# Z2PackDev/TBmodels

Hardware: AMD Instinct MI355X
Metric: k-points/sec (H(k)+eig) at N_orb=64, N_R=4096 (higher is better)
Workload: dtype f64; 1 GPU; cfg2: dense N_orb=64 N_R=4096, 100000 random k-points per GPU, eigenval (H(k)+eig); kpoints_per_gpu=100000, collective=none, rccl_ranks=0, eigensolver=auto

## Files before the change

### tbmodels_amd/csrc/tbk_api.hip

```cpp

#include <algorithm>
#include <cmath>
#include <cstdarg>
#include <cstdlib>
#include <cstring>
#include <dlfcn.h>
#include <functional>
#include <new>
#include <vector>

#include "tbk_internal.h"

static thread_local char g_err[1024] = "";

void tbk_set_error(const char* fmt, ...) {
    va_list ap;
    va_start(ap, fmt);
    vsnprintf(g_err, sizeof(g_err), fmt, ap);
    va_end(ap);
}

extern "C" const char* tbk_last_error(void) { return g_err; }
#ifdef TBK_EXPERIMENTS
extern "C" const char* tbk_version(void) { return "tbk 0.1 (gfx950) +experiments"; }
// ... 283 lines not shown
            m->staged_bytes += nnz * (int64_t)(sizeof(int32_t) + 2 * sizeof(double));
            const int kt = tbk_csr_tile_kpoints(n_r);
            if (kt > 0) {
                std::vector<int64_t> sptr;
                std::vector<int32_t> srec_r;
                std::vector<double> srec_v;
                tbk_csr_schedule(m->ncol, kt, cptr, rec_r, rec_v, sptr, srec_r, srec_v);
                m->sched_steps = sptr.back();
                auto upload = [&](void** dst, const void* src, size_t bytes) -> int {
                    TBK_HIP(hipMalloc(dst, std::max<size_t>(bytes, 8)));
                    if (bytes) TBK_HIP(hipMemcpy(*dst, src, bytes, hipMemcpyHostToDevice));
                    m->staged_bytes += (int64_t)bytes;
                    return TBK_OK;
                };
                TBK_CHECK(upload((void**)&m->d_sptr, sptr.data(), sptr.size() * sizeof(int64_t)));
                TBK_CHECK(upload((void**)&m->d_srec_r, srec_r.data(), srec_r.size() * sizeof(int32_t)));
                TBK_CHECK(upload((void**)&m->d_srec_v, srec_v.data(), srec_v.size() * sizeof(double)));
                m->sched_kt = kt;
            }
        }
        return TBK_OK;
    }();
    if (rc != TBK_OK) {
        tbk_model_destroy(m);
        return rc;
    }
    *out = m;
    return TBK_OK;
}

extern "C" void tbk_model_destroy(tbk_model* m) {
    if (!m) return;
    (void)hipSetDevice(m->device);
    hipStream_t streams[] = {m->stream, m->stream_eig, m->stream_ql, m->stream_xl[0], m->stream_xl[1], m->stream_xl[2]};
    for (hipStream_t st : streams)
        if (st) (void)hipStreamSynchronize(st);
    for (hipEvent_t e : m->ev_xl)
        if (e) (void)hipEventDestroy(e);
    for (int b = 0; b < 2; ++b) {
        if (m->ev_hk[b]) (void)hipEventDestroy(m->ev_hk[b]);
        if (m->ev_tri[b]) (void)hipEventDestroy(m->ev_tri[b]);
        if (m->ev_ql[b]) (void)hipEventDestroy(m->ev_ql[b]);
        if (m->ev_out[b]) (void)hipEventDestroy(m->ev_out[b]);
        if (b == 0 && m->ev_sync) (void)hipEventDestroy(m->ev_sync);
    }
    for (auto& ev : m->events) {
        (void)hipEventDestroy(ev.start);
        (void)hipEventDestroy(ev.stop);
    }
    if (m->blas) (void)rocblas_destroy_handle(m->blas);
    if (m->h_stage) (void)hipHostFree(m->h_stage);
    for (hipStream_t st : streams)
        if (st) (void)hipStreamDestroy(st);
    void* ptrs[] = {m->d_R, m->d_colmap, m->d_B, m->d_cptr, m->d_rec_r, m->d_rec_v, m->d_powers, m->d_sptr, m->d_srec_r, m->d_srec_v};
    for (void* p : ptrs)
        if (p) (void)hipFree(p);
    DevBuf* bufs[] = {&m->ws_phase, &m->ws_H, &m->ws_E,   &m->ws_E2,
                      &m->ws_info,  &m->ws_k, &m->ws_pos, &m->ws_out, &m->ws_out2, &m->ws_flag, &m->ws_orb, &m->ws_part, &m->ws_kfold, &m->ws_kline, &m->ws_band, &m->ws_bandmat[0], &m->ws_bandmat[1], &m->ws_H2, &m->ws_split, &m->ws_xl, &m->ws_posraw};
    for (DevBuf* b : bufs) b->release();
    tbk_fold_release(m);
    delete m;
}

extern "C" int tbk_model_set_option(tbk_model* m, int option, int64_t value) {
    TBK_ARG(m != nullptr, "model is NULL");
    TBK_LOCK(m);
    switch (option) {
        case TBK_OPT_EIGENSOLVER:
            TBK_ARG(value >= TBK_EIG_AUTO && value <= TBK_EIG_ROCSOLVER, "unknown eigensolver");
            m->eigensolver = (int)value;
            return TBK_OK;
        case TBK_OPT_K_CHUNK:
            TBK_ARG(value >= 0, "k chunk must be >= 0");
            m->k_chunk = value;
            return TBK_OK;
        case TBK_OPT_TIMING:
            m->timing = value != 0;
            return TBK_OK;
        case TBK_OPT_FOLD:
            m->fold_enabled = value != 0;
            return TBK_OK;
        default:
            tbk_set_error("unknown option %d", option);
            return TBK_ERR_ARGUMENT;
    }
}

extern "C" int tbk_model_info(const tbk_model* m, int* device, int* dim, int* n_orb, int64_t* n_r,
                              int* is_sparse, int64_t* staged_bytes) {
    TBK_ARG(m != nullptr, "model is NULL");
    if (device) *device = m->device;
    if (dim) *dim = m->dim;
    if (n_orb) *n_orb = m->n_orb;
    if (n_r) *n_r = m->n_r;
    if (is_sparse) *is_sparse = m->sparse ? 1 : 0;
    if (staged_bytes) *staged_bytes = m->staged_bytes;
    return TBK_OK;
}

static int64_t choose_chunk(tbk_model* m, int64_t nk, bool with_eig) {
    if (nk <= TBK_BM) return TBK_BM;
    const int64_t n = m->n_orb;
    int64_t per_k = m->k2 * 8 + (with_eig ? n * n * 16 + (int64_t)tbk_eig_scratch_per_k(m) : 0);
    if (per_k < 64) per_k = 64;
    size_t free_b = 0, total_b = 0;
    if (hipMemGetInfo(&free_b, &total_b) != hipSuccess) free_b = size_t(8) << 30;
    free_b += m->ws_H.bytes + m->ws_H2.bytes + m->ws_phase.bytes + m->ws_band.bytes + m->ws_bandmat[0].bytes + m->ws_bandmat[1].bytes +
              m->ws_E.bytes + m->ws_xl.bytes;
    const bool mid = n > 64 && n <= 256;
    int64_t budget = std::min<int64_t>((int64_t)(free_b / 4), int64_t(mid ? 64 : n > 64 ? 24 : 6) << 30);
    int64_t chunk = budget / per_k / TBK_BM * TBK_BM;
    int64_t cap = mid ? 131072 : 32768;
    if (n < 64) cap *= std::min<int64_t>(32, (64 / n) * (64 / n));
    chunk = std::max<int64_t>(TBK_BM, std::min<int64_t>(chunk, cap));
    if (m->k_chunk > 0) chunk = round_up(m->k_chunk, TBK_BM);
    else if (chunk >= 4096) chunk = chunk / 4096 * 4096;
    return std::min(chunk, round_up(nk, TBK_BM));
}

static inline int64_t phase_ld(int64_t nk) { return round_up(nk, TBK_BM); }

static int fill_rows(tbk_model* m, const double* d_k, int64_t nk, int64_t nk_pad, double* d_A) {
    if (m->kdotp)
        return tbk_launch_monomials(m->stream, m->d_powers, m->dim, m->n_r, m->k2, d_k, nk, nk_pad, d_A);
    return tbk_launch_phase(m, d_k, nk, nk_pad, d_A);
}

static int build_h(tbk_model* m, const double* d_A, int64_t nk, int64_t nk_pad, int mode,
                   int convention, const double* d_k, const double* d_pos, double* d_H) {
    if (m->sparse)
        return tbk_launch_hk_csr(m, d_A, nk, nk_pad, mode, convention, d_k, d_pos, d_H);
    return tbk_launch_hk_dense(m, d_A, nk, nk_pad, mode, convention, d_k, d_pos, d_H);
}

extern "C" int tbk_hamilton_device(tbk_model* m, const double* d_k, int64_t nk, int convention,
                                   const double* d_pos, double* d_H) {
    TBK_ARG(m != nullptr, "model is NULL");
    TBK_LOCK(m);
    TBK_ARG(convention == 1 || convention == 2, "convention must be 1 or 2");
    TBK_ARG(nk >= 0, "nk < 0");
    if (nk == 0) return TBK_OK;
    TBK_ARG(d_k && d_H, "k / H is NULL");
    TBK_ARG(convention == 2 || d_pos != nullptr, "convention 1 needs pos");
    TBK_HIP(hipSetDevice(m->device));
    const int64_t chunk = choose_chunk(m, nk, false);
    const size_t nn2 = (size_t)m->n_orb * m->n_orb * 2;
    for (int64_t c0 = 0; c0 < nk; c0 += chunk) {
        const int64_t nkc = std::min(chunk, nk - c0);
        const int64_t nk_pad = phase_ld(nkc);
        TBK_CHECK(m->ws_phase.reserve((size_t)std::max<int64_t>(m->k2, 1) * nk_pad * sizeof(double)));
        double* d_A = m->ws_phase.as<double>();
        const double* kc = d_k + c0 * m->dim;
        const bool own_rows = tbk_hk_inline_phases(m, nkc);
        if (!own_rows) TBK_CHECK(fill_rows(m, kc, nkc, nk_pad, d_A));
        const double* d_orb = nullptr;
        const bool inline_orb = m->h_k_inline != nullptr && m->d_pos_inline != nullptr && nk == 1 && own_rows;
        if (convention == 1 && !inline_orb) {
            TBK_CHECK(m->ws_orb.reserve((size_t)nkc * m->n_orb * 2 * sizeof(double)));
            TBK_CHECK(tbk_launch_orbital_phases(m, kc, d_pos, nkc, m->ws_orb.as<double>()));
            d_orb = m->ws_orb.as<double>();
        }
// ... 853 lines not shown
```

### tbmodels_amd/csrc/tbk_hk_dense.hip

```cpp

#include <algorithm>
#include <cstdlib>
#include <type_traits>

#include "tbk_internal.h"

namespace {

typedef double d4 __attribute__((ext_vector_type(4)));
typedef double d2 __attribute__((ext_vector_type(2)));
typedef __attribute__((address_space(1))) const void* gptr_t;
typedef __attribute__((address_space(3))) void* lptr_t;

constexpr int LDA = TBK_BM + 16;
constexpr int LDB = 2 * TBK_BNP + 16;
constexpr int STAGE_DOUBLES = TBK_BK * (LDA + LDB);

static_assert(TBK_BM == 128 && TBK_BNP == 64 && TBK_BK == 16, "wave decomposition is written for 128x64x16");

struct HkArgs {
    const double* A;
    const double* Bt;
    const int32_t* colmap;
    const double* kpts;
    const int32_t* R;
    int64_t n_r;
    const double* pos;
    double* H;
    int64_t k2;
    int64_t nk;
    int64_t nk_pad;
    int ncol_pad;
    int n_orb;
    int dim;
    int mt_count;
    int nt_count;
    int xcd_rows;
    double* P;
    int splits;
    int unit_grid;
    int64_t p_rows;
    int64_t a_tile_stride;
    int64_t b_tile_stride;
    int rows_per_tile;
    int block_offset;
    int p_tiles;
    int sub_splits;
    double* P2;
    double k_val[TBK_MAX_DIM];
    int k_inline;
    const double* pos_raw;
};

__device__ __forceinline__ double hk_kcomp(const HkArgs& a, int64_t kq, int d) { return a.k_inline ? a.k_val[d] : a.kpts[kq * a.dim + d]; }

template <int MODE, int CONV>
__device__ __forceinline__ void store_element(const HkArgs& a, int64_t kq, int oi, int oj, double re, double im) {
    if (CONV == 1 && oi != oj) {
        d2 ei, ej;
        if (a.k_inline) {
            double di = 0.0, dj = 0.0;
            for (int d = 0; d < a.dim; ++d) {
                di = fma(a.k_val[d], a.pos_raw[oi * a.dim + d], di);
                dj = fma(a.k_val[d], a.pos_raw[oj * a.dim + d], dj);
            }
            double sn, cs;
            sincospi(2.0 * di, &sn, &cs);
            ei = (d2){cs, sn};
            sincospi(2.0 * dj, &sn, &cs);
            ej = (d2){cs, sn};
        } else {
            ei = *reinterpret_cast<const d2*>(a.pos + ((size_t)kq * a.n_orb + oi) * 2);
            ej = *reinterpret_cast<const d2*>(a.pos + ((size_t)kq * a.n_orb + oj) * 2);
        }
        const double cs = ei[0] * ej[0] + ei[1] * ej[1], sn = ei[0] * ej[1] - ei[1] * ej[0];
        const double t = re * cs - im * sn;
        im = re * sn + im * cs;
        re = t;
    }
    double* hk = a.H + (size_t)kq * a.n_orb * a.n_orb * 2;
    *reinterpret_cast<d2*>(hk + ((size_t)oi * a.n_orb + oj) * 2) = (d2){re, im};
    if (MODE == HK_FULL && oi != oj) *reinterpret_cast<d2*>(hk + ((size_t)oj * a.n_orb + oi) * 2) = (d2){re, -im};
}

__device__ __forceinline__ bool tile_of_block(const HkArgs& a, int b, int& mt, int& nt) {
    if (a.xcd_rows == 0) {
        nt = b % a.nt_count;
        mt = b / a.nt_count;
        return mt < a.mt_count;
    }
    const int x = b & 7;
    const int t = b >> 3;
    const int base = a.mt_count >> 3, extra = a.mt_count & 7;
    const int rows = base + (x < extra ? 1 : 0);
    if (t >= rows * a.nt_count) return false;
    const int start = x * base + (x < extra ? x : extra);
    const int full = rows / a.xcd_rows;
    const int per_group = a.xcd_rows * a.nt_count;
    int row;
    if (t < full * per_group) {
        const int g = t / per_group, r = t % per_group;
        row = g * a.xcd_rows + r % a.xcd_rows;
        nt = r / a.xcd_rows;
    } else {
        const int tt = t - full * per_group, rr = rows - full * a.xcd_rows;
        row = full * a.xcd_rows + tt % rr;
        nt = tt / rr;
    }
    mt = start + row;
    return true;
}

template <int MODE, int CONV, bool SPLIT>
__global__ void __launch_bounds__(256, 2) hk_dense_kernel(const HkArgs a) {
    extern __shared__ __attribute__((aligned(16))) double smem[];

    const int unit = (int)blockIdx.x + a.block_offset;
    const int split_y = SPLIT ? unit / a.unit_grid : 0;
    int mt_idx, nt_idx;
    if (!tile_of_block(a, SPLIT ? unit - split_y * a.unit_grid : unit, mt_idx, nt_idx)) return;

    const int tid = threadIdx.x;
    const int lane = tid & 63;
    const int wave = __builtin_amdgcn_readfirstlane(tid >> 6);
    const int wm = wave >> 1;
    const int wn = wave & 1;
    const int l15 = lane & 15;
    const int l4 = lane >> 4;

    const int64_t m0 = (int64_t)mt_idx * a.rows_per_tile;
    const int64_t n0 = (int64_t)nt_idx * TBK_BNP;

    d4 acc[4][2][2];
#pragma unroll
    for (int i = 0; i < 4; ++i)
// ... 481 lines not shown
int gemv_nkv(int64_t nk) {
    int nkv = 1;
    while (nkv < std::min<int64_t>(nk, 32)) nkv *= 2;
    return nkv;
}
int64_t gemv_strip_rows(const tbk_model* m, int64_t slices) {
    const int64_t n_pairs = m->k2 / 2;
    return (2 * ((n_pairs + slices - 1) / slices) + 15) / 16 * 16;
}

void gemv_plan(const tbk_model* m, int64_t nk, int* slices_out, size_t* lds_out) {
    const int nblk = m->ncol_pad / 64;
    const int64_t n_pairs = m->k2 / 2;
    const size_t per_split = (size_t)nk * m->ncol_pad * 2 * sizeof(double);
    const int64_t cap = std::max<int64_t>(1, (int64_t)((size_t(256) << 20) / per_split));
    const int64_t wave_slots = (int64_t)m->n_cu * 8;
    int64_t slices = wave_slots / nblk;
    size_t lds = 80 * 1024;
    const int64_t rows_one_round = slices > 0 ? (m->k2 + slices - 1) / slices : m->k2 + 1;
    if (slices < 1 || nblk * slices * 10 < wave_slots * 9 || rows_one_round > 384 || slices > cap) {
        slices = std::max<int64_t>(m->k2 / 256, std::min<int64_t>(((int64_t)m->n_cu * 32 + nblk - 1) / nblk, n_pairs / 8));
        slices = std::max<int64_t>(1, std::min(cap, slices));
        lds = 16 * 1024;
    }
    slices = std::max<int64_t>(1, std::min(slices, n_pairs / 8));
    if (nblk * slices * 2 <= wave_slots) lds = 16 * 1024;
    if (lds < 64 * 1024) {
        const size_t need = (size_t)4 * gemv_strip_rows(m, slices) * gemv_nkv(nk) * sizeof(double);
        if (need <= size_t(64) * 1024) lds = std::max(lds, need);
    }
    *slices_out = (int)slices;
    *lds_out = lds;
}

}

bool tbk_hk_inline_phases(const tbk_model* m, int64_t nk) {
    if (!tbk_hk_gemv_path(m, nk) || m->kdotp || m->d_R == nullptr) return false;
    int slices;
    size_t lds;
    gemv_plan(m, nk, &slices, &lds);
    return gemv_strip_rows(m, slices) * gemv_nkv(nk) <= (int64_t)(lds / 32);
}

bool tbk_hk_gemv_path(const tbk_model* m, int64_t nk) {
    if (nk < 1 || m->k2 <= 0 || m->sparse) return false;
    if (nk <= 32) return true;
    return nk <= 4096 && m->ncol_pad <= 256 && m->k2 < 16 * TBK_BK;
}

int tbk_launch_hk_dense(tbk_model* m, const double* d_A, int64_t nk, int64_t nk_pad, int mode,
                        int convention, const double* d_k, const double* d_pos, double* d_H) {
    if (nk == 0) return TBK_OK;
    HkArgs a;
    a.A = d_A;
    a.Bt = m->d_B;
    a.colmap = m->d_colmap;
    a.kpts = d_k;
    a.R = m->d_R;
    a.n_r = m->n_r;
    a.pos = d_pos;
    a.H = d_H;
    a.k2 = m->k2;
    a.nk = nk;
    a.nk_pad = nk_pad;
    a.ncol_pad = m->ncol_pad;
    a.n_orb = m->n_orb;
    a.dim = m->dim;
    a.mt_count = (int)((nk + TBK_BM - 1) / TBK_BM);
    a.nt_count = m->ncol_pad / TBK_BNP;
    int grid;
    if (a.mt_count >= 32) {
        a.xcd_rows = 4;
        if (const char* v = tbk_exp_env("TBK_HK_XCD_ROWS")) a.xcd_rows = std::max(1, atoi(v));
        const int max_rows = (a.mt_count + 7) / 8;
        grid = max_rows * a.nt_count * 8;
    } else {
        a.xcd_rows = 0;
        grid = a.mt_count * a.nt_count;
    }
    a.P = nullptr;
    a.splits = 1;
    a.p_rows = 0;
    a.a_tile_stride = TBK_BM;
    a.b_tile_stride = 0;
    a.rows_per_tile = TBK_BM;
    a.block_offset = 0;
    a.p_tiles = 0;
    a.sub_splits = 1;
    a.P2 = nullptr;
    a.unit_grid = 1;
    a.k_inline = 0;
    a.pos_raw = nullptr;
    for (int d = 0; d < TBK_MAX_DIM; ++d) a.k_val[d] = 0.0;
    if (tbk_hk_gemv_path(m, nk)) {
        int slices;
        size_t lds;
        gemv_plan(m, nk, &slices, &lds);
        const size_t per_split = (size_t)nk * a.ncol_pad * 2 * sizeof(double);
        if (m->h_k_inline != nullptr && nk == 1 && d_A == nullptr && tbk_hk_inline_phases(m, 1)) {
            a.k_inline = 1;
            for (int d = 0; d < m->dim; ++d) a.k_val[d] = m->h_k_inline[d];
            a.pos_raw = m->d_pos_inline;
        }
        TBK_ARG(d_A != nullptr || (tbk_hk_inline_phases(m, nk) && (d_k != nullptr || a.k_inline)), "phase rows missing");
        TBK_ARG(convention != 1 || mode == HK_TRI || d_pos != nullptr || (a.k_inline && a.pos_raw != nullptr), "convention 1 needs the orbital phases");
// ... 97 lines not shown
```

### tbmodels_amd/csrc/tbk_internal.h

```cpp
#pragma once

#include <hip/hip_runtime.h>
#include <rocblas/rocblas.h>

#include <atomic>
#include <cstdlib>
#include <cstdint>
#include <cstdio>
#include <functional>
#include <mutex>
#include <string>
#include <vector>

#include "tbk.h"

constexpr int TBK_BM = 128;
constexpr int TBK_BNP = 64;
constexpr int TBK_BK = 16;
constexpr int TBK_CT = 16;
constexpr int TBK_MAX_DIM = 8;

void tbk_set_error(const char* fmt, ...);

#define TBK_HIP(expr)                                                                             \
// ... 61 lines not shown
        return static_cast<T*>(ptr);
    }
};

struct EventPair {
    hipEvent_t start, stop;
    int stage;
};

struct tbk_fold_plan_t {
    bool built = false;
    int dim = 0;
    int64_t n_r = 0;
    int64_t n_rho = 0, n_rho_pad = 0, k2 = 0;
    int capacity = 0;
    std::vector<int32_t> h_R2;
    int32_t* d_R2 = nullptr;
    int64_t* d_lptr = nullptr;
    int32_t* d_lrec = nullptr;
    int32_t* d_rcomp = nullptr;
    double* d_B2 = nullptr;
    double* d_table = nullptr;
    int64_t table_entries = 0;
    tbk_fold_plan_t* sub = nullptr;
};

struct tbk_fold_saved_t {
    int dim;
    int64_t n_r, n_r_pad, k2;
    int32_t* d_R;
    double* d_B;
};

struct tbk_model {
    std::recursive_mutex mu;
    int device = 0;
    int64_t call_nk = 0;
    int n_cu = 256;
    int dim = 0;
    int n_orb = 0;
    int64_t n_r = 0;
    bool sparse = false;
    bool kdotp = false;

    int64_t n_r_pad = 0;
    int64_t k2 = 0;
    int ncol = 0;
    int ncol_pad = 0;
    int32_t* d_R = nullptr;
    int32_t* d_colmap = nullptr;
    int32_t* d_powers = nullptr;

    double* d_B = nullptr;

    int64_t nnz_rec = 0;
    int64_t* d_cptr = nullptr;
    int32_t* d_rec_r = nullptr;
    double* d_rec_v = nullptr;
    int sched_kt = 0;
    int64_t sched_steps = 0;
    int64_t* d_sptr = nullptr;
    int32_t* d_srec_r = nullptr;
    double* d_srec_v = nullptr;

    int64_t staged_bytes = 0;

    std::vector<int32_t> h_R;
    tbk_fold_plan_t fold[TBK_MAX_DIM];
    bool fold_enabled = true;
    int64_t counters[TBK_CNT_COUNT] = {0, 0, 0, 0};

    int eigensolver = TBK_EIG_AUTO;
    int64_t k_chunk = 0;
    bool timing = false;

    hipStream_t stream = nullptr;
    hipStream_t stream_eig = nullptr;
    hipStream_t stream_ql = nullptr;
    hipStream_t stream_xl[3] = {nullptr, nullptr, nullptr};
    hipEvent_t ev_xl[4] = {nullptr, nullptr, nullptr, nullptr};
    hipEvent_t ev_hk[2] = {nullptr, nullptr};
    hipEvent_t ev_tri[2] = {nullptr, nullptr};
    hipEvent_t ev_out[2] = {nullptr, nullptr};
    hipEvent_t ev_ql[2] = {nullptr, nullptr};
    hipEvent_t ev_sync = nullptr;
    rocblas_handle blas = nullptr;
    DevBuf ws_phase;
    DevBuf ws_H;
    DevBuf ws_H2;
    DevBuf ws_E;
    DevBuf ws_E2;
    DevBuf ws_info;
    DevBuf ws_k;
    DevBuf ws_pos;
    DevBuf ws_orb;
    DevBuf ws_out;
    DevBuf ws_out2;
    DevBuf ws_flag;
    void* h_stage = nullptr;
    size_t h_stage_bytes = 0;
    DevBuf ws_part;
    DevBuf ws_kfold;
    DevBuf ws_kline;
    DevBuf ws_band;
    DevBuf ws_bandmat[2];
    const double* h_k_inline = nullptr;
    const double* d_pos_inline = nullptr;
    std::vector<double> pos_cache;
    DevBuf ws_posraw;
    DevBuf ws_split;
    DevBuf ws_xl;
    std::function<int(int64_t c0, int64_t nkc, hipEvent_t done)> chunk_done;
    size_t hk_lds_floor = 0;
    std::vector<EventPair> events;
    double t_ms[TBK_T_COUNT] = {0, 0, 0, 0};
    int64_t t_n[TBK_T_COUNT] = {0, 0, 0, 0};
};

struct tbk_kdotp {
    tbk_model* core = nullptr;
};

void tbk_range_push(const char* name);
void tbk_range_pop();

struct StageTimer {
    tbk_model* m;
    EventPair ev;
    bool on;
    hipStream_t stream;
    StageTimer(tbk_model* m_, int stage, hipStream_t s = nullptr);
    ~StageTimer();
};

enum HkMode { HK_TRI = 0, HK_FULL = 1 };

int tbk_launch_phase(tbk_model* m, const double* d_k, int64_t nk, int64_t nk_pad, double* d_A);
int tbk_launch_orbital_phases(tbk_model* m, const double* d_k, const double* d_pos, int64_t nk, double* d_orb);
int tbk_launch_monomials(hipStream_t s, const int32_t* d_powers, int dim, int64_t n_p,
                         int64_t n_p_pad, const double* d_k, int64_t nk, int64_t nk_pad,
                         double* d_A);

int tbk_stage_dense(tbk_model* m, const double* d_hop_raw);
int tbk_stage_kdotp(tbk_model* m, const double* d_coeff_raw);

int tbk_launch_hk_dense(tbk_model* m, const double* d_A, int64_t nk, int64_t nk_pad, int mode,
                        int convention, const double* d_k, const double* d_pos, double* d_H);

int tbk_launch_hk_dense_lines(tbk_model* m, const double* d_A, int64_t n_lines, int line_len, int64_t b_stride, double* d_H);

int tbk_launch_hk_csr(tbk_model* m, const double* d_A, int64_t nk, int64_t nk_pad, int mode,
                      int convention, const double* d_k, const double* d_pos, double* d_H);

int tbk_csr_tile_kpoints(int64_t n_r);
void tbk_csr_schedule(int ncol, int kt, const std::vector<int64_t>& cptr, const std::vector<int32_t>& rec_r, const std::vector<double>& rec_v,
                      std::vector<int64_t>& sptr, std::vector<int32_t>& srec_r, std::vector<double>& srec_v);

int tbk_eig_batched(tbk_model* m, double* d_H, int64_t nk, double* d_E);

bool tbk_eig_stream_supported(int n);
int tbk_launch_tridiag_stream(tbk_model* m, hipStream_t s, double* d_H, int64_t nk, double* d_de, int method = 0);
bool tbk_hk_inline_phases(const tbk_model* m, int64_t nk);
bool tbk_hk_gemv_path(const tbk_model* m, int64_t nk);
int tbk_launch_bisect(tbk_model* m, hipStream_t s, const double* d_de, int64_t nk, double* d_E);
size_t tbk_eig_scratch_per_k(const tbk_model* m);
int tbk_band_xl_reserve(tbk_model* m, int64_t max_nk);

bool tbk_eig_band_supported(int n);
bool tbk_eig_band_preferred(int n);
size_t tbk_band_scratch_per_matrix(int n);
size_t tbk_band_bytes_per_matrix(int n);
size_t tbk_band_xl_buffer_per_matrix(int n);
bool tbk_eig_two_stage(const tbk_model* m);
int tbk_launch_band_reduce(tbk_model* m, hipStream_t s, double* d_H, int64_t nk, void* d_vw, void* d_band,
                           double* d_de_fused = nullptr);
bool tbk_band_fused(int n);
bool tbk_band_split(const tbk_model* m, int64_t nk);
bool tbk_band_xl_grouped(int n, int64_t nk);
int tbk_launch_band_chase(tbk_model* m, hipStream_t s, const void* d_band, int64_t nk, double* d_de);

bool tbk_eig_small_supported(int n);
int tbk_launch_tridiag(tbk_model* m, hipStream_t s, double* d_H, int64_t nk, double* d_de);
bool tbk_eig_reg128_supported(int n);
int tbk_launch_tridiag_reg128(hipStream_t s, double* d_H, int n, int64_t nk, double* d_D, double* d_E, int64_t h_stride, int ldd, int off);
int tbk_launch_tridiag_tail64(hipStream_t s, double* d_H, int64_t nk, double* d_D, double* d_E, int n_full, int64_t call_nk);
int tbk_launch_ql(tbk_model* m, hipStream_t s, const double* d_de, int64_t nk, double* d_E, bool beside_ql = false);

int tbk_fold_choose(tbk_model* m, const double* h_k, int64_t nk, std::vector<int64_t>& run_starts);
int tbk_fold_group_size();
int tbk_fold_group(tbk_model* m, tbk_fold_plan_t& plan, const double* h_kf, int n_g, int slot0);
int tbk_fold_lines(tbk_model* m, tbk_fold_plan_t& plan, const double* d_kf, int64_t stride, int n_lines, int slot0 = 0);
int tbk_fold_enter(tbk_model* m, tbk_fold_plan_t& plan, int slot, tbk_fold_saved_t& saved);
void tbk_fold_leave(tbk_model* m, const tbk_fold_saved_t& saved);
int tbk_fold_drop_component(tbk_model* m, const double* d_k, int dim, int f, int64_t nk, double* d_k2);
int tbk_fold_subplan(tbk_model* m, tbk_fold_plan_t& parent, int f2, int capacity, tbk_fold_plan_t** out);
void tbk_fold_release(tbk_model* m);
int64_t tbk_fold_min_run();

int tbk_run_mfma_f64_peak(double* tflops);
```

### tbmodels_amd/csrc/tbk_phase.hip

```cpp

#include "tbk_internal.h"

namespace {

__global__ void __launch_bounds__(256)
phase_rows_kernel(const double* __restrict__ k, const int32_t* __restrict__ R, int dim, int64_t nk,
                  int64_t nk_pad, int64_t n_r, double* __restrict__ A) {
    const int64_t kidx = (int64_t)blockIdx.x * blockDim.x + threadIdx.x;
    const int64_t r = blockIdx.y;
    if (kidx >= nk_pad) return;
    double c = 0.0, s = 0.0;
    if (kidx < nk && r < n_r) {
        double dot = 0.0;
        for (int d = 0; d < dim; ++d)
            dot = fma(k[kidx * dim + d], (double)R[r * dim + d], dot);
        sincospi(2.0 * dot, &s, &c);
    }
    A[(2 * r) * nk_pad + kidx] = c;
    A[(2 * r + 1) * nk_pad + kidx] = s;
}

__global__ void __launch_bounds__(256)
monomial_rows_kernel(const double* __restrict__ k, const int32_t* __restrict__ powers, int dim,
                     int64_t nk, int64_t nk_pad, int64_t n_p, double* __restrict__ A) {
    const int64_t kidx = (int64_t)blockIdx.x * blockDim.x + threadIdx.x;
    const int64_t p = blockIdx.y;
    if (kidx >= nk_pad) return;
    double v = 0.0;
    if (kidx < nk && p < n_p) {
        v = 1.0;
        for (int d = 0; d < dim; ++d) {
            const double x = k[kidx * dim + d];
            const int e = powers[p * dim + d];
            double acc = 1.0;
            for (int t = 0; t < e; ++t) acc *= x;
            v *= acc;
        }
    }
    A[p * nk_pad + kidx] = v;
}

__global__ void __launch_bounds__(256)
orbital_phase_kernel(const double* __restrict__ k, const double* __restrict__ pos, int dim, int64_t nk,
                     int n_orb, double* __restrict__ orb) {
    const int64_t idx = (int64_t)blockIdx.x * blockDim.x + threadIdx.x;
    if (idx >= nk * n_orb) return;
    const int64_t kq = idx / n_orb;
    const int p = (int)(idx % n_orb);
    double dot = 0.0;
    for (int d = 0; d < dim; ++d) dot = fma(k[kq * dim + d], pos[p * dim + d], dot);
    double s, c;
    sincospi(2.0 * dot, &s, &c);
    orb[2 * idx] = c;
    orb[2 * idx + 1] = s;
}

}

int tbk_launch_orbital_phases(tbk_model* m, const double* d_k, const double* d_pos, int64_t nk, double* d_orb) {
    if (nk == 0) return TBK_OK;
    const int64_t total = nk * m->n_orb;
    hipLaunchKernelGGL(orbital_phase_kernel, dim3((unsigned)((total + 255) / 256)), dim3(256), 0, m->stream, d_k,
                       d_pos, m->dim, nk, m->n_orb, d_orb);
    TBK_HIP(hipGetLastError());
    return TBK_OK;
}

int tbk_launch_phase(tbk_model* m, const double* d_k, int64_t nk, int64_t nk_pad, double* d_A) {
    if (m->n_r_pad == 0 || nk_pad == 0) return TBK_OK;
    StageTimer t(m, TBK_T_PHASE);
    dim3 grid((unsigned)((nk_pad + 255) / 256), (unsigned)m->n_r_pad);
    hipLaunchKernelGGL(phase_rows_kernel, grid, dim3(256), 0, m->stream, d_k, m->d_R, m->dim, nk,
                       nk_pad, m->n_r, d_A);
    TBK_HIP(hipGetLastError());
    return TBK_OK;
}

int tbk_launch_monomials(hipStream_t s, const int32_t* d_powers, int dim, int64_t n_p,
                         int64_t n_p_pad, const double* d_k, int64_t nk, int64_t nk_pad,
                         double* d_A) {
    if (n_p_pad == 0 || nk_pad == 0) return TBK_OK;
    dim3 grid((unsigned)((nk_pad + 255) / 256), (unsigned)n_p_pad);
    hipLaunchKernelGGL(monomial_rows_kernel, grid, dim3(256), 0, s, d_k, d_powers, dim, nk, nk_pad,
                       n_p, d_A);
    TBK_HIP(hipGetLastError());
    return TBK_OK;
}
```

### tbmodels_amd/csrc/tbk_stage.hip

```cpp

#include "tbk_internal.h"

namespace {

__global__ void __launch_bounds__(256)
stage_dense_kernel(const double* __restrict__ hop, const int32_t* __restrict__ colmap, int n_orb,
                   int64_t n_r, int ncol_pad, double* __restrict__ Bt) {
    const int e = blockIdx.x * blockDim.x + threadIdx.x;
    const int64_t r = blockIdx.y;
    if (e >= ncol_pad || r >= n_r) return;
    const int32_t ij = colmap[e];
    if (ij < 0) return;
    const int i = ij >> 16, j = ij & 0xffff;
    const double* blk = hop + (size_t)r * n_orb * n_orb * 2;
    const double hr = blk[((size_t)i * n_orb + j) * 2], hi = blk[((size_t)i * n_orb + j) * 2 + 1];
    const double gr = blk[((size_t)j * n_orb + i) * 2], gi = blk[((size_t)j * n_orb + i) * 2 + 1];
    const size_t tiles = ncol_pad / TBK_CT;
    const size_t base0 = (((size_t)(2 * r) * tiles + e / TBK_CT) * 2) * TBK_CT + e % TBK_CT;
    const size_t base1 = (((size_t)(2 * r + 1) * tiles + e / TBK_CT) * 2) * TBK_CT + e % TBK_CT;
    Bt[base0] = hr + gr;
    Bt[base0 + TBK_CT] = hi - gi;
    Bt[base1] = -(hi + gi);
    Bt[base1 + TBK_CT] = hr - gr;
}

__global__ void __launch_bounds__(256)
stage_kdotp_kernel(const double* __restrict__ coeff, const int32_t* __restrict__ colmap, int n_orb,
                   int64_t n_p, int ncol_pad, double* __restrict__ Bt) {
    const int e = blockIdx.x * blockDim.x + threadIdx.x;
    const int64_t p = blockIdx.y;
    if (e >= ncol_pad || p >= n_p) return;
    const int32_t ij = colmap[e];
    if (ij < 0) return;
    const int i = ij >> 16, j = ij & 0xffff;
    const double* blk = coeff + (size_t)p * n_orb * n_orb * 2;
    const size_t tiles = ncol_pad / TBK_CT;
    const size_t base = (((size_t)p * tiles + e / TBK_CT) * 2) * TBK_CT + e % TBK_CT;
    Bt[base] = blk[((size_t)i * n_orb + j) * 2];
    Bt[base + TBK_CT] = blk[((size_t)i * n_orb + j) * 2 + 1];
}

}

int tbk_stage_dense(tbk_model* m, const double* d_hop_raw) {
    const size_t bytes = (size_t)m->k2 * m->ncol_pad * 2 * sizeof(double);
    if (bytes == 0) return TBK_OK;
    TBK_HIP(hipMalloc((void**)&m->d_B, bytes));
    m->staged_bytes += (int64_t)bytes;
    TBK_HIP(hipMemsetAsync(m->d_B, 0, bytes, m->stream));
    if (m->n_r > 0) {
        TBK_ARG(m->n_r <= 65535, "more than 65535 lattice vectors");
        dim3 grid((m->ncol_pad + 255) / 256, (unsigned)m->n_r);
        hipLaunchKernelGGL(stage_dense_kernel, grid, dim3(256), 0, m->stream, d_hop_raw, m->d_colmap,
                           m->n_orb, m->n_r, m->ncol_pad, m->d_B);
        TBK_HIP(hipGetLastError());
    }
    return TBK_OK;
}

int tbk_stage_kdotp(tbk_model* m, const double* d_coeff_raw) {
    const size_t bytes = (size_t)m->k2 * m->ncol_pad * 2 * sizeof(double);
    if (bytes == 0) return TBK_OK;
    TBK_HIP(hipMalloc((void**)&m->d_B, bytes));
    m->staged_bytes += (int64_t)bytes;
    TBK_HIP(hipMemsetAsync(m->d_B, 0, bytes, m->stream));
    if (m->n_r > 0) {
        TBK_ARG(m->n_r <= 65535, "more than 65535 Taylor coefficients");
        dim3 grid((m->ncol_pad + 255) / 256, (unsigned)m->n_r);
        hipLaunchKernelGGL(stage_kdotp_kernel, grid, dim3(256), 0, m->stream, d_coeff_raw,
                           m->d_colmap, m->n_orb, m->n_r, m->ncol_pad, m->d_B);
        TBK_HIP(hipGetLastError());
    }
    return TBK_OK;
}
```

Baseline: 961,000 k-points/s.

## Emulate the FP64 H(k) GEMM with int8 MFMA over sixteen CRT moduli

```diff
diff --git a/tbmodels_amd/csrc/tbk_api.hip b/tbmodels_amd/csrc/tbk_api.hip
--- a/tbmodels_amd/csrc/tbk_api.hip
+++ b/tbmodels_amd/csrc/tbk_api.hip
@@ -359,11 +359,11 @@
     if (m->h_stage) (void)hipHostFree(m->h_stage);
     for (hipStream_t st : streams)
         if (st) (void)hipStreamDestroy(st);
-    void* ptrs[] = {m->d_R, m->d_colmap, m->d_B, m->d_cptr, m->d_rec_r, m->d_rec_v, m->d_powers, m->d_sptr, m->d_srec_r, m->d_srec_v};
+    void* ptrs[] = {m->d_R, m->d_colmap, m->d_B, m->d_Bres, m->d_bexp, m->d_cptr, m->d_rec_r, m->d_rec_v, m->d_powers, m->d_sptr, m->d_srec_r, m->d_srec_v};
     for (void* p : ptrs)
         if (p) (void)hipFree(p);
     DevBuf* bufs[] = {&m->ws_phase, &m->ws_H, &m->ws_E,   &m->ws_E2,
-                      &m->ws_info,  &m->ws_k, &m->ws_pos, &m->ws_out, &m->ws_out2, &m->ws_flag, &m->ws_orb, &m->ws_part, &m->ws_kfold, &m->ws_kline, &m->ws_band, &m->ws_bandmat[0], &m->ws_bandmat[1], &m->ws_H2, &m->ws_split, &m->ws_xl, &m->ws_posraw};
+                      &m->ws_info,  &m->ws_k, &m->ws_pos, &m->ws_out, &m->ws_out2, &m->ws_flag, &m->ws_orb, &m->ws_part, &m->ws_kfold, &m->ws_kline, &m->ws_band, &m->ws_bandmat[0], &m->ws_bandmat[1], &m->ws_H2, &m->ws_split, &m->ws_xl, &m->ws_posraw, &m->ws_ares, &m->ws_planes};
     for (DevBuf* b : bufs) b->release();
     tbk_fold_release(m);
     delete m;
@@ -413,7 +413,7 @@
     size_t free_b = 0, total_b = 0;
     if (hipMemGetInfo(&free_b, &total_b) != hipSuccess) free_b = size_t(8) << 30;
     free_b += m->ws_H.bytes + m->ws_H2.bytes + m->ws_phase.bytes + m->ws_band.bytes + m->ws_bandmat[0].bytes + m->ws_bandmat[1].bytes +
-              m->ws_E.bytes + m->ws_xl.bytes;
+              m->ws_E.bytes + m->ws_xl.bytes + m->ws_ares.bytes + m->ws_planes.bytes;
     const bool mid = n > 64 && n <= 256;
     int64_t budget = std::min<int64_t>((int64_t)(free_b / 4), int64_t(mid ? 64 : n > 64 ? 24 : 6) << 30);
     int64_t chunk = budget / per_k / TBK_BM * TBK_BM;
diff --git a/tbmodels_amd/csrc/tbk_hk_dense.hip b/tbmodels_amd/csrc/tbk_hk_dense.hip
--- a/tbmodels_amd/csrc/tbk_hk_dense.hip
+++ b/tbmodels_amd/csrc/tbk_hk_dense.hip
@@ -56,8 +56,8 @@
 
 template <int MODE, int CONV>
 __device__ __forceinline__ void store_element(const HkArgs& a, int64_t kq, int oi, int oj, double re, double im) {
+    d2 ei = (d2){1.0, 0.0}, ej = (d2){1.0, 0.0};
     if (CONV == 1 && oi != oj) {
-        d2 ei, ej;
         if (a.k_inline) {
             double di = 0.0, dj = 0.0;
             for (int d = 0; d < a.dim; ++d) {
@@ -73,14 +73,8 @@
             ei = *reinterpret_cast<const d2*>(a.pos + ((size_t)kq * a.n_orb + oi) * 2);
             ej = *reinterpret_cast<const d2*>(a.pos + ((size_t)kq * a.n_orb + oj) * 2);
         }
-        const double cs = ei[0] * ej[0] + ei[1] * ej[1], sn = ei[0] * ej[1] - ei[1] * ej[0];
-        const double t = re * cs - im * sn;
-        im = re * sn + im * cs;
-        re = t;
-    }
-    double* hk = a.H + (size_t)kq * a.n_orb * a.n_orb * 2;
-    *reinterpret_cast<d2*>(hk + ((size_t)oi * a.n_orb + oj) * 2) = (d2){re, im};
-    if (MODE == HK_FULL && oi != oj) *reinterpret_cast<d2*>(hk + ((size_t)oj * a.n_orb + oi) * 2) = (d2){re, -im};
+    }
+    tbk_store_h_element<MODE, CONV>(a.H, a.n_orb, kq, oi, oj, re, im, ei[0], ei[1], ej[0], ej[1]);
 }
 
 __device__ __forceinline__ bool tile_of_block(const HkArgs& a, int b, int& mt, int& nt) {
@@ -668,6 +662,7 @@
 int tbk_launch_hk_dense(tbk_model* m, const double* d_A, int64_t nk, int64_t nk_pad, int mode,
                         int convention, const double* d_k, const double* d_pos, double* d_H) {
     if (nk == 0) return TBK_OK;
+    if (tbk_hk_i8_route(m, nk)) return tbk_launch_hk_i8(m, d_k, nk, mode, convention, d_pos, d_H);
     HkArgs a;
     a.A = d_A;
     a.Bt = m->d_B;
diff --git a/tbmodels_amd/csrc/tbk_hk_i8.hip b/tbmodels_amd/csrc/tbk_hk_i8.hip
--- /dev/null
+++ b/tbmodels_amd/csrc/tbk_hk_i8.hip
@@ -0,0 +1,369 @@
+
+#include <cmath>
+#include <cstdlib>
+
+#include "tbk_internal.h"
+
+namespace {
+
+__constant__ int c_mod[TBK_I8_NMOD] = {256, 255, 253, 251, 247, 241, 239, 233, 229, 227, 223, 217, 211, 199, 197, 193};
+constexpr int H_MOD[TBK_I8_NMOD] = {256, 255, 253, 251, 247, 241, 239, 233, 229, 227, 223, 217, 211, 199, 197, 193};
+constexpr int ALPHA = 52;
+
+typedef int v4i __attribute__((ext_vector_type(4)));
+typedef int v16i __attribute__((ext_vector_type(16)));
+typedef double d2 __attribute__((ext_vector_type(2)));
+
+constexpr int I8_BN = 128;
+constexpr int I8_LDR = 80;
+constexpr int I8_STAGE = (TBK_I8_BM + I8_BN) * I8_LDR;
+static_assert(TBK_I8_BM == 256 && TBK_I8_BK == 64, "wave decomposition is written for 256 x 128 x 64");
+
+constexpr int modinv(int a, int p) {
+    a %= p;
+    for (int x = 1; x < p; ++x)
+        if ((a * x) % p == 1) return x;
+    return 0;
+}
+
+template <int P>
+__device__ __forceinline__ int sym(int r) {
+    return 2 * r >= P ? r - P : r;
+}
+
+__device__ __forceinline__ int sym_mod_f64(double x, int p) {
+    const double q = floor(x * (1.0 / (double)p));
+    int r = (int)fma(-q, (double)p, x);
+    if (r < 0) r += p;
+    if (r >= p) r -= p;
+    return 2 * r >= p ? r - p : r;
+}
+
+__global__ void __launch_bounds__(256)
+i8_stage_kernel(const double* __restrict__ Bt, int nc, int64_t k2, int64_t kpad, int beta, int8_t* __restrict__ Bres,
+                int32_t* __restrict__ bexp, int* __restrict__ nonfinite) {
+    __shared__ double s_max[256];
+    const int c = blockIdx.x;
+    double mx = 0.0;
+    bool bad = false;
+    for (int64_t kk = threadIdx.x; kk < k2; kk += 256) {
+        const double v = Bt[kk * nc + c];
+        mx = fmax(mx, fabs(v));
+        bad |= !isfinite(v);
+    }
+    if (bad) atomicAdd(nonfinite, 1);
+    s_max[threadIdx.x] = mx;
+    __syncthreads();
+    for (int w = 128; w > 0; w >>= 1) {
+        if (threadIdx.x < w) s_max[threadIdx.x] = fmax(s_max[threadIdx.x], s_max[threadIdx.x + w]);
+        __syncthreads();
+    }
+    mx = s_max[0];
+    int ex = 0;
+    if (mx > 0.0) (void)frexp(mx, &ex);
+    const int bc = mx > 0.0 ? beta - ex : 0;
+    if (threadIdx.x == 0) bexp[c] = bc;
+    for (int64_t kk = threadIdx.x; kk < kpad; kk += 256) {
+        const double v = kk < k2 && mx > 0.0 ? rint(ldexp(Bt[kk * nc + c], bc)) : 0.0;
+        const int64_t iv = isfinite(v) ? (int64_t)v : 0;
+#pragma unroll
+        for (int i = 0; i < TBK_I8_NMOD; ++i) {
+            const int p = c_mod[i];
+            int r = (int)(iv % p);
+            if (r < 0) r += p;
+            Bres[((int64_t)i * nc + c) * kpad + kk] = (int8_t)(2 * r >= p ? r - p : r);
+        }
+    }
+}
+
+__global__ void __launch_bounds__(256)
+i8_rows_kernel(const double* __restrict__ k, const int32_t* __restrict__ R, int dim, int64_t nk, int64_t n_r, int64_t mpad,
+               int64_t kpad, int8_t* __restrict__ Ares, int* __restrict__ row_bad) {
+    const int64_t r = (int64_t)blockIdx.x * blockDim.x + threadIdx.x;
+    const int64_t m = blockIdx.y;
+    if (2 * r >= kpad) return;
+    double c = 0.0, s = 0.0;
+    if (m < nk && r < n_r) {
+        double dot = 0.0;
+        for (int d = 0; d < dim; ++d) dot = fma(k[m * dim + d], (double)R[r * dim + d], dot);
+        sincospi(2.0 * dot, &s, &c);
+        if (!isfinite(c) || !isfinite(s)) {
+            row_bad[m] = 1;
+            c = s = 0.0;
+        }
+    }
+    const double ca = rint(ldexp(c, ALPHA)), sa = rint(ldexp(s, ALPHA));
+#pragma unroll
+    for (int i = 0; i < TBK_I8_NMOD; ++i) {
+        const int p = c_mod[i];
+        const uint32_t lo = (uint32_t)(uint8_t)(int8_t)sym_mod_f64(ca, p), hi = (uint32_t)(uint8_t)(int8_t)sym_mod_f64(sa, p);
+        *reinterpret_cast<uint16_t*>(Ares + ((int64_t)i * mpad + m) * kpad + 2 * r) = (uint16_t)(lo | (hi << 8));
+    }
+}
+
+template <int I>
+__device__ __forceinline__ int mod_pick(int x, int z) {
+    if constexpr (I == TBK_I8_NMOD) {
+        return 0;
+    } else {
+        if (z == I) {
+            int r = x % H_MOD[I];
+            return r < 0 ? r + H_MOD[I] : r;
+        }
+        return mod_pick<I + 1>(x, z);
+    }
+}
+
+__global__ void __launch_bounds__(256, 2)
+hk_i8_gemm_kernel(const int8_t* __restrict__ Ares, const int8_t* __restrict__ Bres, uint8_t* __restrict__ planes, int64_t mpad,
+                  int nc, int64_t kpad, int nt_count) {
+    extern __shared__ __attribute__((aligned(16))) char smem_i8[];
+    const int z = blockIdx.z;
+    const int mt = blockIdx.x / nt_count, nt = blockIdx.x - mt * nt_count;
+    const int tid = threadIdx.x, lane = tid & 63;
+    const int wave = __builtin_amdgcn_readfirstlane(tid >> 6);
+    const int wm = wave >> 1, wn = wave & 1;
+    const int l31 = lane & 31, l5 = lane >> 5;
+
+    const int8_t* gA = Ares + ((int64_t)z * mpad + (int64_t)mt * TBK_I8_BM) * kpad;
+    const int8_t* gB = Bres + ((int64_t)z * nc + (int64_t)nt * I8_BN) * kpad;
+    const int prow = tid >> 2, ppart = (tid & 3) * 16;
+    v4i ra[4], rb[2];
+    auto fetch = [&](int64_t kb) {
+#pragma unroll
+        for (int s = 0; s < 4; ++s) ra[s] = *reinterpret_cast<const v4i*>(gA + (int64_t)(prow + 64 * s) * kpad + kb + ppart);
+#pragma unroll
+        for (int s = 0; s < 2; ++s) rb[s] = *reinterpret_cast<const v4i*>(gB + (int64_t)(prow + 64 * s) * kpad + kb + ppart);
+    };
+    auto put = [&](int buf) {
+        char* sA = smem_i8 + buf * I8_STAGE;
+        char* sB = sA + TBK_I8_BM * I8_LDR;
+#pragma unroll
+        for (int s = 0; s < 4; ++s) *reinterpret_cast<v4i*>(sA + (prow + 64 * s) * I8_LDR + ppart) = ra[s];
+#pragma unroll
+        for (int s = 0; s < 2; ++s) *reinterpret_cast<v4i*>(sB + (prow + 64 * s) * I8_LDR + ppart) = rb[s];
+    };
+
+    v16i acc[4][2];
+#pragma unroll
+    for (int i = 0; i < 4; ++i)
+#pragma unroll
+        for (int j = 0; j < 2; ++j)
+#pragma unroll
+            for (int r = 0; r < 16; ++r) acc[i][j][r] = 0;
+
+    const int n_stage = (int)(kpad / TBK_I8_BK);
+    fetch(0);
+    put(0);
+    __syncthreads();
+    for (int st = 0; st < n_stage; ++st) {
+        const int buf = st & 1;
+        if (st + 1 < n_stage) fetch((int64_t)(st + 1) * TBK_I8_BK);
+        const char* sA = smem_i8 + buf * I8_STAGE + (wm * 128 + l31) * I8_LDR + l5 * 16;
+        const char* sB = smem_i8 + buf * I8_STAGE + TBK_I8_BM * I8_LDR + (wn * 64 + l31) * I8_LDR + l5 * 16;
+#pragma unroll
+        for (int ks = 0; ks < 2; ++ks) {
+            v4i fa[4], fb[2];
+#pragma unroll
+            for (int i = 0; i < 4; ++i) fa[i] = *reinterpret_cast<const v4i*>(sA + i * 32 * I8_LDR + ks * 32);
+#pragma unroll
+            for (int j = 0; j < 2; ++j) fb[j] = *reinterpret_cast<const v4i*>(sB + j * 32 * I8_LDR + ks * 32);
+#pragma unroll
+            for (int i = 0; i < 4; ++i)
+#pragma unroll
+                for (int j = 0; j < 2; ++j) acc[i][j] = __builtin_amdgcn_mfma_i32_32x32x32_i8(fa[i], fb[j], acc[i][j], 0, 0, 0);
+        }
+        if (st + 1 < n_stage) put(buf ^ 1);
+        __syncthreads();
+    }
+
+    uint8_t* out = planes + ((int64_t)z * mpad + (int64_t)mt * TBK_I8_BM + wm * 128) * nc + (int64_t)nt * I8_BN + wn * 64;
+#pragma unroll
+    for (int i = 0; i < 4; ++i)
+#pragma unroll
+        for (int j = 0; j < 2; ++j)
+#pragma unroll
+            for (int r = 0; r < 16; ++r)
+                out[(int64_t)(i * 32 + (r & 3) + 8 * (r >> 2) + 4 * l5) * nc + j * 32 + l31] = (uint8_t)mod_pick<0>(acc[i][j][r], z);
+}
+
+template <int I, int J>
+__device__ __forceinline__ int garner_inner(int t, const int (&v)[TBK_I8_NMOD]) {
+    if constexpr (J == I) {
+        return t;
+    } else {
+        constexpr int P = H_MOD[I];
+        constexpr int INV = modinv(H_MOD[J], P);
+        return garner_inner<I, J + 1>(((t - v[J] + P) * INV) % P, v);
+    }
+}
+
+template <int I>
+__device__ __forceinline__ void garner_step(const int (&x)[TBK_I8_NMOD], int (&v)[TBK_I8_NMOD]) {
+    if constexpr (I < TBK_I8_NMOD) {
+        v[I] = sym<H_MOD[I]>(garner_inner<I, 0>(x[I], v));
+        garner_step<I + 1>(x, v);
+    }
+}
+
+__device__ __forceinline__ double reconstruct(const uint8_t* __restrict__ pl, int64_t plane_stride) {
+    int x[TBK_I8_NMOD], v[TBK_I8_NMOD];
+#pragma unroll
+    for (int i = 0; i < TBK_I8_NMOD; ++i) x[i] = pl[i * plane_stride];
+    garner_step<0>(x, v);
+    double s = (double)v[TBK_I8_NMOD - 1];
+#pragma unroll
+    for (int i = TBK_I8_NMOD - 2; i >= 0; --i) s = fma(s, (double)H_MOD[i], (double)v[i]);
+    return s;
+}
+
+template <int MODE, int CONV>
+__global__ void __launch_bounds__(256)
+hk_i8_recon_kernel(const uint8_t* __restrict__ planes, const int32_t* __restrict__ bexp, const int32_t* __restrict__ colmap,
+                   const int* __restrict__ row_bad, const double* __restrict__ pos, int64_t mpad, int nc, int ncol_pad, int n_orb,
+                   double* __restrict__ H) {
+    const int e = blockIdx.x * blockDim.x + threadIdx.x;
+    const int64_t kq = blockIdx.y;
+    if (e >= ncol_pad) return;
+    const int32_t ij = colmap[e];
+    if (ij < 0) return;
+    const int oi = ij >> 16, oj = ij & 0xffff;
+    const int c_re = (e >> 4) * 32 + (e & 15), c_im = c_re + 16;
+    const int64_t ps = mpad * nc;
+    const uint8_t* row = planes + kq * nc;
+    double re = ldexp(reconstruct(row + c_re, ps), -(ALPHA + bexp[c_re]));
+    double im = ldexp(reconstruct(row + c_im, ps), -(ALPHA + bexp[c_im]));
+    if (row_bad[kq]) re = im = __builtin_nan("");
+    d2 ei = (d2){1.0, 0.0}, ej = (d2){1.0, 0.0};
+    if (CONV == 1 && oi != oj) {
+        ei = *reinterpret_cast<const d2*>(pos + ((size_t)kq * n_orb + oi) * 2);
+        ej = *reinterpret_cast<const d2*>(pos + ((size_t)kq * n_orb + oj) * 2);
+    }
+    tbk_store_h_element<MODE, CONV>(H, n_orb, kq, oi, oj, re, im, ei[0], ei[1], ej[0], ej[1]);
+}
+
+inline int64_t round_up_i8(int64_t x, int64_t m) { return (x + m - 1) / m * m; }
+
+}
+
+static bool i8_enabled() {
+    static const bool on = !(getenv("TBK_HK_INT8") && atoi(getenv("TBK_HK_INT8")) == 0);
+    return on;
+}
+
+constexpr int64_t I8_MIN_K = 1024;
+constexpr int64_t I8_MIN_ROWS = 8192;
+constexpr int64_t I8_WS_BYTES = int64_t(8) << 30;
+
+int tbk_stage_i8(tbk_model* m) {
+    if (m->kdotp || m->sparse || m->d_B == nullptr || m->k2 < I8_MIN_ROWS || !i8_enabled()) return TBK_OK;
+    const int nc = m->ncol_pad * 2;
+    const int64_t kpad = round_up_i8(m->k2, TBK_I8_BK);
+    if (kpad * 128 * 128 >= (int64_t(1) << 31)) return TBK_OK;
+    double log2p = 0.0;
+    for (int i = 0; i < TBK_I8_NMOD; ++i) log2p += std::log2((double)H_MOD[i]);
+    const int beta = std::min(62, (int)std::floor(log2p - 1.0 - ALPHA - std::log2((double)kpad) - 1e-9));
+    if (beta < 1) return TBK_OK;
+    int8_t* d_res = nullptr;
+    int32_t* d_exp = nullptr;
+    const size_t bytes = (size_t)TBK_I8_NMOD * nc * kpad;
+    if (hipMalloc((void**)&d_res, bytes) != hipSuccess || hipMalloc((void**)&d_exp, (size_t)nc * sizeof(int32_t) + sizeof(int)) != hipSuccess) {
+        (void)hipGetLastError();
+        if (d_res) (void)hipFree(d_res);
+        return TBK_OK;
+    }
+    int* d_flag = reinterpret_cast<int*>(d_exp + nc);
+    int flag = 0;
+    const int rc = [&]() -> int {
+        TBK_HIP(hipMemsetAsync(d_flag, 0, sizeof(int), m->stream));
+        hipLaunchKernelGGL(i8_stage_kernel, dim3((unsigned)nc), dim3(256), 0, m->stream, m->d_B, nc, m->k2, kpad, beta, d_res, d_exp,
+                           d_flag);
+        TBK_HIP(hipGetLastError());
+        TBK_HIP(hipMemcpyAsync(&flag, d_flag, sizeof(int), hipMemcpyDeviceToHost, m->stream));
+        TBK_HIP(hipStreamSynchronize(m->stream));
+        return TBK_OK;
+    }();
+    if (rc != TBK_OK || flag != 0) {
+        (void)hipFree(d_res);
+        (void)hipFree(d_exp);
+        return rc;
+    }
+    m->d_Bres = d_res;
+    m->d_bexp = d_exp;
+    m->i8_k = kpad;
+    m->i8_src = m->d_B;
+    m->staged_bytes += (int64_t)bytes;
+    return TBK_OK;
+}
+
+bool tbk_hk_i8_route(const tbk_model* m, int64_t nk) {
+    return nk >= I8_MIN_K && m->k2 >= I8_MIN_ROWS && !tbk_hk_gemv_path(m, nk) && m->d_Bres != nullptr && m->d_B == m->i8_src &&
+           round_up_i8(m->k2, TBK_I8_BK) == m->i8_k && !m->sparse && !m->kdotp && i8_enabled();
+}
+
+static int64_t i8_piece(const tbk_model* m) {
+    const int64_t per_k = (int64_t)TBK_I8_NMOD * (m->i8_k + 2 * (int64_t)m->ncol_pad) + (int64_t)sizeof(int);
+    return std::max<int64_t>(TBK_I8_BM, std::min<int64_t>(32768, I8_WS_BYTES / per_k / TBK_I8_BM * TBK_I8_BM));
+}
+
+static int i8_rows(tbk_model* m, const double* d_k, int64_t nk) {
+    const int64_t mpad = round_up_i8(nk, TBK_I8_BM);
+    const size_t rows_bytes = (size_t)TBK_I8_NMOD * mpad * m->i8_k;
+    TBK_CHECK(m->ws_ares.reserve(rows_bytes + (size_t)mpad * sizeof(int)));
+    int* row_bad = reinterpret_cast<int*>(m->ws_ares.as<char>() + rows_bytes);
+    StageTimer t(m, TBK_T_PHASE);
+    TBK_HIP(hipMemsetAsync(row_bad, 0, (size_t)mpad * sizeof(int), m->stream));
+    dim3 grid((unsigned)((m->i8_k / 2 + 255) / 256), (unsigned)mpad);
+    hipLaunchKernelGGL(i8_rows_kernel, grid, dim3(256), 0, m->stream, d_k, m->d_R, m->dim, nk, m->n_r, mpad, m->i8_k,
+                       m->ws_ares.as<int8_t>(), row_bad);
+    TBK_HIP(hipGetLastError());
+    m->ares_k = d_k;
+    m->ares_nk = nk;
+    return TBK_OK;
+}
+
+int tbk_launch_i8_rows(tbk_model* m, const double* d_k, int64_t nk) {
+    return nk <= i8_piece(m) ? i8_rows(m, d_k, nk) : TBK_OK;
+}
+
+int tbk_launch_hk_i8(tbk_model* m, const double* d_k, int64_t nk, int mode, int convention, const double* d_pos, double* d_H) {
+    TBK_ARG(d_k != nullptr, "int8 route: k-points missing");
+    TBK_ARG(convention != 1 || d_pos != nullptr, "convention 1 needs the orbital phases");
+    const int64_t piece = i8_piece(m);
+    const int nc = m->ncol_pad * 2;
+    const size_t nn2 = (size_t)m->n_orb * m->n_orb * 2;
+    static tbk_flag_row lds_done;
+    const int lds = 2 * I8_STAGE;
+    TBK_HIP(tbk_raise_lds_limit((const void*)hk_i8_gemm_kernel, lds, lds_done));
+    for (int64_t p0 = 0; p0 < nk; p0 += piece) {
+        const int64_t np = std::min(piece, nk - p0);
+        const double* kp = d_k + p0 * m->dim;
+        if (m->ares_k != kp || m->ares_nk != np) TBK_CHECK(i8_rows(m, kp, np));
+        m->ares_k = nullptr;
+        m->ares_nk = -1;
+        const int64_t mpad = round_up_i8(np, TBK_I8_BM);
+        const int* row_bad = reinterpret_cast<const int*>(m->ws_ares.as<char>() + (size_t)TBK_I8_NMOD * mpad * m->i8_k);
+        TBK_CHECK(m->ws_planes.reserve((size_t)TBK_I8_NMOD * mpad * nc));
+        StageTimer t(m, TBK_T_HK);
+        const int nt_count = nc / I8_BN;
+        const dim3 grid((unsigned)((mpad / TBK_I8_BM) * nt_count), 1, TBK_I8_NMOD);
+        hipLaunchKernelGGL(hk_i8_gemm_kernel, grid, dim3(256), lds, m->stream, m->ws_ares.as<int8_t>(), m->d_Bres,
+                           m->ws_planes.as<uint8_t>(), mpad, nc, m->i8_k, nt_count);
+        TBK_HIP(hipGetLastError());
+        const dim3 grid_r((unsigned)((m->ncol_pad + 255) / 256), (unsigned)np);
+        const uint8_t* pl = m->ws_planes.as<uint8_t>();
+        double* hp = d_H + (size_t)p0 * nn2;
+        const double* pp = d_pos ? d_pos + (size_t)p0 * m->n_orb * 2 : nullptr;
+        if (mode == HK_TRI)
+            hipLaunchKernelGGL((hk_i8_recon_kernel<HK_TRI, 2>), grid_r, dim3(256), 0, m->stream, pl, m->d_bexp, m->d_colmap, row_bad,
+                               pp, mpad, nc, m->ncol_pad, m->n_orb, hp);
+        else if (convention == 1)
+            hipLaunchKernelGGL((hk_i8_recon_kernel<HK_FULL, 1>), grid_r, dim3(256), 0, m->stream, pl, m->d_bexp, m->d_colmap, row_bad,
+                               pp, mpad, nc, m->ncol_pad, m->n_orb, hp);
+        else
+            hipLaunchKernelGGL((hk_i8_recon_kernel<HK_FULL, 2>), grid_r, dim3(256), 0, m->stream, pl, m->d_bexp, m->d_colmap, row_bad,
+                               pp, mpad, nc, m->ncol_pad, m->n_orb, hp);
+        TBK_HIP(hipGetLastError());
+    }
+    return TBK_OK;
+}
diff --git a/tbmodels_amd/csrc/tbk_internal.h b/tbmodels_amd/csrc/tbk_internal.h
--- a/tbmodels_amd/csrc/tbk_internal.h
+++ b/tbmodels_amd/csrc/tbk_internal.h
@@ -137,6 +137,10 @@
     int32_t* d_powers = nullptr;
 
     double* d_B = nullptr;
+    int8_t* d_Bres = nullptr;
+    int32_t* d_bexp = nullptr;
+    int64_t i8_k = 0;
+    const double* i8_src = nullptr;
 
     int64_t nnz_rec = 0;
     int64_t* d_cptr = nullptr;
@@ -184,6 +188,10 @@
     DevBuf ws_flag;
     void* h_stage = nullptr;
     size_t h_stage_bytes = 0;
+    DevBuf ws_ares;
+    DevBuf ws_planes;
+    const double* ares_k = nullptr;
+    int64_t ares_nk = -1;
     DevBuf ws_part;
     DevBuf ws_kfold;
     DevBuf ws_kline;
@@ -220,6 +228,21 @@
 
 enum HkMode { HK_TRI = 0, HK_FULL = 1 };
 
+typedef double tbk_d2 __attribute__((ext_vector_type(2)));
+template <int MODE, int CONV>
+__device__ __forceinline__ void tbk_store_h_element(double* H, int n_orb, int64_t kq, int oi, int oj, double re, double im, double eic,
+                                                    double eis, double ejc, double ejs) {
+    if (CONV == 1 && oi != oj) {
+        const double cs = eic * ejc + eis * ejs, sn = eic * ejs - eis * ejc;
+        const double t = re * cs - im * sn;
+        im = re * sn + im * cs;
+        re = t;
+    }
+    double* hk = H + (size_t)kq * n_orb * n_orb * 2;
+    *reinterpret_cast<tbk_d2*>(hk + ((size_t)oi * n_orb + oj) * 2) = (tbk_d2){re, im};
+    if (MODE == HK_FULL && oi != oj) *reinterpret_cast<tbk_d2*>(hk + ((size_t)oj * n_orb + oi) * 2) = (tbk_d2){re, -im};
+}
+
 int tbk_launch_phase(tbk_model* m, const double* d_k, int64_t nk, int64_t nk_pad, double* d_A);
 int tbk_launch_orbital_phases(tbk_model* m, const double* d_k, const double* d_pos, int64_t nk, double* d_orb);
 int tbk_launch_monomials(hipStream_t s, const int32_t* d_powers, int dim, int64_t n_p,
@@ -233,6 +256,14 @@
                         int convention, const double* d_k, const double* d_pos, double* d_H);
 
 int tbk_launch_hk_dense_lines(tbk_model* m, const double* d_A, int64_t n_lines, int line_len, int64_t b_stride, double* d_H);
+
+constexpr int TBK_I8_NMOD = 16;
+constexpr int TBK_I8_BM = 256;
+constexpr int TBK_I8_BK = 64;
+int tbk_stage_i8(tbk_model* m);
+bool tbk_hk_i8_route(const tbk_model* m, int64_t nk);
+int tbk_launch_i8_rows(tbk_model* m, const double* d_k, int64_t nk);
+int tbk_launch_hk_i8(tbk_model* m, const double* d_k, int64_t nk, int mode, int convention, const double* d_pos, double* d_H);
 
 int tbk_launch_hk_csr(tbk_model* m, const double* d_A, int64_t nk, int64_t nk_pad, int mode,
                       int convention, const double* d_k, const double* d_pos, double* d_H);
diff --git a/tbmodels_amd/csrc/tbk_phase.hip b/tbmodels_amd/csrc/tbk_phase.hip
--- a/tbmodels_amd/csrc/tbk_phase.hip
+++ b/tbmodels_amd/csrc/tbk_phase.hip
@@ -68,6 +68,7 @@
 
 int tbk_launch_phase(tbk_model* m, const double* d_k, int64_t nk, int64_t nk_pad, double* d_A) {
     if (m->n_r_pad == 0 || nk_pad == 0) return TBK_OK;
+    if (tbk_hk_i8_route(m, nk)) return tbk_launch_i8_rows(m, d_k, nk);
     StageTimer t(m, TBK_T_PHASE);
     dim3 grid((unsigned)((nk_pad + 255) / 256), (unsigned)m->n_r_pad);
     hipLaunchKernelGGL(phase_rows_kernel, grid, dim3(256), 0, m->stream, d_k, m->d_R, m->dim, nk,
diff --git a/tbmodels_amd/csrc/tbk_stage.hip b/tbmodels_amd/csrc/tbk_stage.hip
--- a/tbmodels_amd/csrc/tbk_stage.hip
+++ b/tbmodels_amd/csrc/tbk_stage.hip
@@ -55,7 +55,7 @@
                            m->n_orb, m->n_r, m->ncol_pad, m->d_B);
         TBK_HIP(hipGetLastError());
     }
-    return TBK_OK;
+    return tbk_stage_i8(m);
 }
 
 int tbk_stage_kdotp(tbk_model* m, const double* d_coeff_raw) {
```

Measured after the change: 1.018 million k-points/s (median of 6 runs). 1.06x the previous value.
